# foundation-model-stack/fms-fsdp

Hardware: AMD Instinct MI355X
Metric: tokens/sec (aggregate) (higher is better)
Workload: dtype bf16; 1 GPU; model=llama2_7b, global_batch=2, seq_len=4096, parallelism=hsdp1

## Files before the change

fms_fsdp_amd/ops/hip/attention.hip:

```cpp
#include <cstdlib>
#include <cstring>

#include "common.h"
#include "attn_sched.h"
#include "attn_ws.h"

typedef __attribute__((ext_vector_type(8))) __bf16 bf16x8v;
typedef __attribute__((ext_vector_type(16))) float f32x16;
typedef __attribute__((ext_vector_type(4))) float f32x4v;

union U8 {
  bf16x8v v;
  unsigned u[4];
  bf16x8 s;
};

__device__ __forceinline__ unsigned pack2(float lo, float hi) {
  return ((unsigned)(unsigned short)f2bf(hi) << 16) |
         (unsigned short)f2bf(lo);
}

__device__ __forceinline__ bf16x8v pack_pT_chunk(const float* p) {
  unsigned w01 = pack2(p[0], p[1]);
  unsigned w23 = pack2(p[2], p[3]);
// ... 257 lines not shown
        pb1_1 = pack_pT_chunk(p + 8);
      }
    }
    __syncthreads();
    if (tile + 1 < ntiles) stage_k();
    if (act1) {
      const unsigned pvbase = pvb[cur] + 1024;
      U2x64 fr[2][2];
      tr_issue4<0, 128, 512, 640>(pvbase, fr[0][0], fr[0][1]);
#pragma unroll
      for (int t = 0; t < NT; ++t) {
        const int pp = t & 1;
        if (t + 1 < NT) {
          if (t + 1 == 1)
            tr_issue4<4096, 4096 + 128, 4096 + 512, 4096 + 640>(
                pvbase, fr[1][0], fr[1][1]);
          else if (t + 1 == 2)
            tr_issue4<8192, 8192 + 128, 8192 + 512, 8192 + 640>(
                pvbase, fr[0][0], fr[0][1]);
          else
            tr_issue4<12288, 12288 + 128, 12288 + 512, 12288 + 640>(
                pvbase, fr[1][0], fr[1][1]);
          tr_wait<4>(fr[pp][0], fr[pp][1]);
        } else {
          tr_wait<0>(fr[pp][0], fr[pp][1]);
        }
        accO[t] = __builtin_amdgcn_mfma_f32_32x32x16_bf16(fr[pp][0].v, pb1_0,
                                                          accO[t], 0, 0, 0);
        accO[t] = __builtin_amdgcn_mfma_f32_32x32x16_bf16(fr[pp][1].v, pb1_1,
                                                          accO[t], 0, 0, 0);
      }
    }
    __syncthreads();
    cur ^= 1;
  }

  const float inv_l = 1.f / l_run;
  short* op = og + ((long long)b * S * H + (long long)h) * D +
              (long long)my_q * qrow_stride;
#pragma unroll
  for (int t = 0; t < NT; ++t) {
#pragma unroll
    for (int g = 0; g < 4; ++g) {
      const int dv0 = t * 32 + 8 * g + 4 * hb;
      bf16x4 w;
#pragma unroll
      for (int j = 0; j < 4; ++j)
        w.v[j] = f2bf(accO[t][g * 4 + j] * inv_l);
      *(bf16x4*)(op + dv0) = w;
    }
  }
  if (hb == 0)
    lseg[((long long)bh) * S + my_q] =
        (m_run + __log2f(l_run)) * 0.6931471805599453f;
}
#undef KLDS
#undef VLDS

__global__ void attn_bwd_delta_kernel(const short* __restrict__ dog,
                                      const short* __restrict__ og,
                                      float* __restrict__ delta,
                                      int D, int S, int H, long long rows) {
  const long long row = ((long long)blockIdx.x * blockDim.x + threadIdx.x) / 64;
  if (row >= rows) return;
  const int lane = threadIdx.x & 63;
  const short* dop = dog + row * D;
  const short* op = og + row * D;
  float acc = 0.f;
  for (int i = lane * 2; i < D; i += 128) {
    acc += bf2f(dop[i]) * bf2f(op[i]) + bf2f(dop[i + 1]) * bf2f(op[i + 1]);
  }
  acc = wave_reduce_sum(acc);
  if (lane == 0) {
    const long long b = row / ((long long)S * H);
    const int si = (int)((row / H) % S);
    const int hi = (int)(row % H);
    delta[(b * H + hi) * (long long)S + si] = acc;
  }
}

template <int D>
__global__ __launch_bounds__(256, 2) void attn_bwd_dq_kernel(
    const short* __restrict__ kg, const short* __restrict__ dsw,
    short* __restrict__ dqg, int B, int S, int H, int KVH, int sched) {
  constexpr int KVB = 32;
  constexpr int NT = D / 32;
  extern __shared__ __attribute__((aligned(16))) char smem[];
  constexpr int KIMGB = KVB * D * 2;
  constexpr int SIMGB = KVB * 128 * 2;
#define KIMG(buf) (smem + ((buf) ? KIMGB + SIMGB : 0))
#define SIMG(buf) (smem + KIMGB + ((buf) ? KIMGB + SIMGB : 0))

  const int lane = threadIdx.x & 63;
  const int wid = threadIdx.x >> 6;
  const int col = lane & 31;
  const int hb = lane >> 5;

  const AttnWork wk = attn_sched_map(blockIdx.x, S / 128, B * H, sched, false);
  const int bh = __builtin_amdgcn_readfirstlane(wk.bh);
  const int b = bh / H;
  const int h = bh % H;
  const int kvh = h / (H / KVH);
  const int q0 = __builtin_amdgcn_readfirstlane(wk.tile) * 128;
  const int qw = q0 + wid * 32;
  const int my_q = qw + col;

  const long long qrow_stride = (long long)H * D;
  const long long krow_stride = (long long)KVH * D;
  const short* kbase = kg + ((long long)b * S * KVH + (long long)kvh) * D;
  const short* dsbase = dsw + (long long)bh * S * S + q0;

  f32x16 accDQ[NT];
#pragma unroll
  for (int t = 0; t < NT; ++t) accDQ[t] = (f32x16)(0.f);

  const int ntiles = (q0 + 128 + KVB - 1) / KVB;
  const int t256 = threadIdx.x;
  const int skey = t256 & 31;
  const int sgrp = t256 >> 5;
  const int skd0 = sgrp * (D / 8);
  const short* kp_s = kbase + (long long)skey * krow_stride + skd0;
  const long long kstep = (long long)KVB * krow_stride;
  const short* sp_s = dsbase + (long long)skey * S + sgrp * 16;
  const long long sstep = (long long)KVB * S;
  const int koff = SUBT_OFF(skey, skd0, 8);
  const int koff1 = SUBT_OFF(skey, skd0 + 8, 8);
  const int soff0 = SUBT_OFF(skey, sgrp * 16, 8);
  const int soff1 = SUBT_OFF(skey, sgrp * 16 + 8, 8);
  auto stage = [&](int buf) {
    if constexpr (D == 128) {
      *(f32x4*)(KIMG(buf) + koff) = *(const f32x4*)(kp_s);
      *(f32x4*)(KIMG(buf) + koff1) = *(const f32x4*)(kp_s + 8);
    } else {
      *(f32x4*)(KIMG(buf) + koff) = *(const f32x4*)(kp_s);
    }
    *(f32x4*)(SIMG(buf) + soff0) = *(const f32x4*)(sp_s);
    *(f32x4*)(SIMG(buf) + soff1) = *(const f32x4*)(sp_s + 8);
    kp_s += kstep;
    sp_s += sstep;
  };
  stage(0);
  __syncthreads();
  const unsigned ktr = tr_base<1024>(lane, col, hb);
  const unsigned kib[2] = {(unsigned)(unsigned long long)KIMG(0) + ktr,
                           (unsigned)(unsigned long long)KIMG(1) + ktr};
  const unsigned str = (unsigned)((((lane & 15) * 8) ^ (16 * hb)) +
                                  hb * 256 + ((col >> 4) << 10) +
                                  (wid * 32) * 64);
  const unsigned sib[2] = {(unsigned)(unsigned long long)SIMG(0) + str,
                           (unsigned)(unsigned long long)SIMG(1) + str};

  int cur = 0;
  for (int tile = 0; tile < ntiles; ++tile) {
    if (tile + 1 < ntiles) stage(cur ^ 1);
    U2x64 bs[2];
    tr_issue4<0, 128, 512, 512 + 128>(sib[cur], bs[0], bs[1]);
    tr_wait<0>(bs[0], bs[1]);
    const unsigned kbase_t = kib[cur];
    U2x64 fr[2][2];
    tr_issue4<0, 128, 512, 640>(kbase_t, fr[0][0], fr[0][1]);
#pragma unroll
    for (int t = 0; t < NT; ++t) {
      const int pp = t & 1;
      if (t + 1 < NT) {
        if (t + 1 == 1)
          tr_issue4<2048, 2048 + 128, 2048 + 512, 2048 + 640>(
              kbase_t, fr[1][0], fr[1][1]);
        else if (t + 1 == 2)
          tr_issue4<4096, 4096 + 128, 4096 + 512, 4096 + 640>(
              kbase_t, fr[0][0], fr[0][1]);
        else
          tr_issue4<6144, 6144 + 128, 6144 + 512, 6144 + 640>(
              kbase_t, fr[1][0], fr[1][1]);
        tr_wait<4>(fr[pp][0], fr[pp][1]);
      } else {
        tr_wait<0>(fr[pp][0], fr[pp][1]);
      }
      accDQ[t] = __builtin_amdgcn_mfma_f32_32x32x16_bf16(fr[pp][0].v,
                                                         bs[0].v, accDQ[t],
                                                         0, 0, 0);
      accDQ[t] = __builtin_amdgcn_mfma_f32_32x32x16_bf16(fr[pp][1].v,
                                                         bs[1].v, accDQ[t],
                                                         0, 0, 0);
    }
    __syncthreads();
    cur ^= 1;
  }

  short* dqp = dqg + ((long long)b * S * H + (long long)h) * D +
               (long long)my_q * qrow_stride;
#pragma unroll
  for (int t = 0; t < NT; ++t) {
#pragma unroll
    for (int g = 0; g < 4; ++g) {
      const int dk0 = t * 32 + 8 * g + 4 * hb;
      bf16x4 w;
#pragma unroll
      for (int j = 0; j < 4; ++j) w.v[j] = f2bf(accDQ[t][g * 4 + j]);
      *(bf16x4*)(dqp + dk0) = w;
    }
  }
}
#undef KIMG
#undef SIMG

template <int D>
// ... 283 lines not shown
      const int key = DROW(r, hb);
      *(short*)(my_p + key * 80 + col * 2) = f2bf(pv[r]);
    }
#define DKV_TRLOOP(ACC, A0, A1, BASE)                                        \
  do {                                                                       \
    _Pragma("unroll") for (int t = 0; t < NT; ++t) {                         \
      U2x64 f0, f1;                                                          \
      const unsigned b_t = (BASE) + t * 2048;                                \
      tr_issue4<0, 128, 512, 640>(b_t, f0, f1);                              \
      tr_wait<0>(f0, f1);                                                    \
      ACC[t] = __builtin_amdgcn_mfma_f32_32x32x16_bf16(A0, f0.v, ACC[t],     \
                                                       0, 0, 0);             \
      ACC[t] = __builtin_amdgcn_mfma_f32_32x32x16_bf16(A1, f1.v, ACC[t],     \
                                                       0, 0, 0);             \
    }                                                                        \
  } while (0)
    {
      bf16x8v pa[2];
#pragma unroll
      for (int kc = 0; kc < 2; ++kc) {
        const int inrow = kc * 32 + hb * 16;
        pa[kc] = *(const bf16x8v*)(my_p + col * 80 + inrow);
      }
      const unsigned dob = (unsigned)(unsigned long long)DOIMG(cur) + kv_swz;
      DKV_TRLOOP(accDV, pa[0], pa[1], dob);
    }
#pragma unroll
    for (int r = 0; r < 16; ++r) {
      const int key = DROW(r, hb);
      *(short*)(my_p + key * 80 + col * 2) = f2bf(ds[r]);
    }
    if constexpr (PUBLISH_DS) {
      const int key = lane & 31;
      const long long grow = ((long long)bh * S + kv0 + key) * S + q0;
#pragma unroll
      for (int c = 0; c < 2; ++c) {
        const int qc = ((lane >> 5) * 2 + c) * 8;
        *(f32x4*)(dsw + grow + qc) =
            *(const f32x4*)(my_p + key * 80 + qc * 2);
      }
    }
    {
      bf16x8v da[2];
#pragma unroll
      for (int kc = 0; kc < 2; ++kc) {
        const int inrow = kc * 32 + hb * 16;
        da[kc] = *(const bf16x8v*)(my_p + col * 80 + inrow);
      }
      const unsigned qib = (unsigned)(unsigned long long)QIMG(cur) + kv_swz;
      DKV_TRLOOP(accDK, da[0], da[1], qib);
    }
#undef DKV_TRLOOP
    __syncthreads();
    cur ^= 1;
  }
#undef QIMG
#undef DOIMG

#pragma unroll
  for (int t = 0; t < NT; ++t) {
#pragma unroll
    for (int r = 0; r < 16; ++r) {
      const int key_abs = kv0 + DROW(r, hb);
      const int feat = t * 32 + col;
      const long long off =
          ((long long)b * S + key_abs) * (long long)(KVH * D) +
          (long long)kvh * D + feat;
      const long long offv = ((long long)b * S + key_abs) * dvstride +
                             (long long)kvh * D + feat;
      if (OUT_BF16) {
        ((short*)dkg)[off] = f2bf(accDK[t][r]);
        ((short*)dvg)[offv] = f2bf(accDV[t][r]);
      } else if (ngrp > 1) {
        atomicAdd((float*)dkg + off, accDK[t][r]);
        atomicAdd((float*)dvg + offv, accDV[t][r]);
      } else {
        ((float*)dkg)[off] += accDK[t][r];
        ((float*)dvg)[offv] += accDV[t][r];
      }
    }
  }
}

static int g_attn_sched = -1;

static int attn_sched_get() {
  if (g_attn_sched < 0) {
    const char* e = getenv("FMS_AMD_ATTN_SCHED");
    g_attn_sched = (e && strcmp(e, "legacy") == 0) ? ATTN_SCHED_LEGACY
                                                   : ATTN_SCHED_BALANCED;
  }
  return g_attn_sched;
}

static long long g_attn_ws_limit = -1;

static long long attn_ws_limit_get() {
  if (g_attn_ws_limit < 0) {
    long long mb = ATTN_BWD_WS_DEFAULT_MB;
    const char* e = getenv("FMS_AMD_ATTN_BWD_WS_MB");
    if (e && *e) {
      char* end = nullptr;
      const long long val = strtoll(e, &end, 10);
      if (end != e && *end == '\0' && val >= 0 && val <= (1LL << 40)) mb = val;
    }
    g_attn_ws_limit = mb << 20;
  }
  return g_attn_ws_limit;
}

template <int D>
static void attn_bwd_launch(const void* do_, const void* q, const void* k,
                            const void* v, const float* lse, void* dq,
                            void* dk, void* dv, float* delta_ws, void* ds_ws,
                            int B, int S, int H, int KVH, float scale,
                            int out_bf16, long long vstride,
                            long long dvstride, hipStream_t stream) {
  const unsigned grid = (unsigned)(S / 128) * (unsigned)(B * H);
  const int sched = attn_sched_get();
  const int lds_dkv = 4 * 32 * D * 2 + 4 * 32 * D * 2 + 4 * 32 * 80;
#define DKV_LAUNCH(OUT, PUB)                                                  \
  attn_bwd_dkv_kernel<D, OUT, PUB><<<grid, 256, lds_dkv, stream>>>(           \
      (const short*)do_, (const short*)q, (const short*)k, (const short*)v,   \
      lse, delta_ws, dk, dv, (short*)ds_ws, B, S, H, KVH, scale, vstride,     \
      dvstride, sched)
  if (ds_ws) {
    if (out_bf16)
      DKV_LAUNCH(true, true);
    else
      DKV_LAUNCH(false, true);
    const int lds_dq = 2 * (32 * D * 2 + 32 * 128 * 2);
    attn_bwd_dq_kernel<D><<<grid, 256, lds_dq, stream>>>(
        (const short*)k, (const short*)ds_ws, (short*)dq, B, S, H, KVH, sched);
  } else {
    if (out_bf16)
      DKV_LAUNCH(true, false);
    else
      DKV_LAUNCH(false, false);
    const int lds_dq = 2 * (32 * D * 2 + 32 * D * 2);
    attn_bwd_dq_recompute_kernel<D><<<grid, 256, lds_dq, stream>>>(
        (const short*)do_, (const short*)q, (const short*)k, (const short*)v,
        lse, delta_ws, (short*)dq, B, S, H, KVH, scale, vstride, sched);
  }
#undef DKV_LAUNCH
}

extern "C" {

long long attn_bwd_ws_limit(long long bytes) {
  const long long prev = attn_ws_limit_get();
  if (bytes >= 0) g_attn_ws_limit = bytes;
  return prev;
}

int attn_sched_mode(int mode) {
  const int prev = attn_sched_get();
  if (mode >= 0) g_attn_sched = mode;
  return prev;
}

void launch_attn_fwd(const void* q, const void* k, const void* v, void* o,
                     float* lse, int B, int S, int H, int KVH, int D,
                     float scale, long long vstride, hipStream_t stream) {
  const unsigned grid = (unsigned)(S / 128) * (unsigned)(B * H);
  const int sched = attn_sched_get();
  const int lds = 3 * 64 * D * 2;
  if (D == 128)
    attn_fwd_kernel<128><<<grid, 256, lds, stream>>>(
        (const short*)q, (const short*)k, (const short*)v, (short*)o, lse, B,
        S, H, KVH, scale, vstride, sched);
  else
    attn_fwd_kernel<64><<<grid, 256, lds, stream>>>(
        (const short*)q, (const short*)k, (const short*)v, (short*)o, lse, B,
        S, H, KVH, scale, vstride, sched);
}

void launch_attn_bwd(const void* do_, const void* q, const void* k,
                     const void* v, const void* o, const float* lse, void* dq,
                     void* dk, void* dv, float* delta_ws, void* ds_ws,
                     int B, int S, int H,
                     int KVH, int D, float scale, int out_bf16,
                     long long vstride, long long dvstride,
                     hipStream_t stream) {
  const long long rows = (long long)B * S * H;
  attn_bwd_delta_kernel<<<(int)((rows * 64 + 255) / 256), 256, 0, stream>>>(
      (const short*)do_, (const short*)o, delta_ws, D, S, H, rows);
  if (D == 128)
    attn_bwd_launch<128>(do_, q, k, v, lse, dq, dk, dv, delta_ws, ds_ws, B, S,
                         H, KVH, scale, out_bf16, vstride, dvstride, stream);
  else
    attn_bwd_launch<64>(do_, q, k, v, lse, dq, dk, dv, delta_ws, ds_ws, B, S,
                        H, KVH, scale, out_bf16, vstride, dvstride, stream);
}

}
```

fms_fsdp_amd/ops/hip/bindings.cpp:

```cpp
#include <torch/extension.h>
#include <c10/hip/HIPStream.h>
#include <hip/hip_runtime_api.h>

#include <string>
#include <tuple>
#include <vector>

#include "attn_ws.h"

using torch::Tensor;

extern "C" {
void launch_rmsnorm_fwd(const void*, const void*, void*, float*, int, int,
                        float, hipStream_t);
void launch_rmsnorm_bwd(const void*, const void*, const void*, const float*,
                        const void*, void*, float*, int, int, hipStream_t);
void launch_add_rmsnorm_fwd(const void*, const void*, const void*, void*,
                            void*, float*, int, int, float, hipStream_t);
void launch_rope(const void*, void*, const float*, const float*, int, int,
                 int, int, int, long long, long long, hipStream_t);
void launch_swiglu_fwd(const void*, void*, long long, int, hipStream_t);
void launch_swiglu_bwd(const void*, const void*, void*, long long, int,
                       hipStream_t);
void launch_ce_fwd_bwd(void*, const long long*, float*, const float*,
                       long long, int, int, hipStream_t);
void launch_adamw(float*, const void*, int, float*, float*, void*, int,
                  long long, float, float, float, float, float, float, float,
                  const float*, hipStream_t);
void launch_sqnorm(const void*, int, float*, long long, hipStream_t);
void launch_attn_fwd(const void*, const void*, const void*, void*, float*,
                     int, int, int, int, int, float, long long, hipStream_t);
void launch_attn_bwd(const void*, const void*, const void*, const void*,
                     const void*, const float*, void*, void*, void*, float*,
                     void*, int, int, int, int, int, float, int,
                     long long, long long, hipStream_t);
int attn_sched_mode(int);
long long attn_bwd_ws_limit(long long);
void launch_cconv_fwd(const void*, const void*, const float*, void*, int,
                      int, int, int, hipStream_t);
void launch_cconv_bwd(const void*, const void*, const void*, const float*,
                      void*, void*, float*, float*, int, int, int, int,
                      hipStream_t);
int launch_gemm_nt(const void*, const void*, void*, int, int, int,
                   hipStream_t);
void launch_segsum_exp_fwd(const float*, void*, long long, int, hipStream_t);
void launch_segsum_exp_bwd(const void*, const float*, float*, long long, int,
                           hipStream_t);
void launch_ssd_prep_fwd(const void*, const float*, const float*, float*,
                         float*, long long, int, int, long long, hipStream_t);
void launch_ssd_prep_bwd(const float*, const float*, const void*,
                         const float*, const float*, void*, float*, float*,
                         long long, int, int, long long, long long,
                         hipStream_t);
void launch_ssd_xdt_fwd(const void*, const float*, const float*, void*, void*,
                        long long, int, int, int, long long, hipStream_t);
void launch_ssd_xdt_bwd(const void*, const void*, const void*, const float*,
                        const float*, void*, float*, float*, long long, int,
                        int, int, long long, long long, hipStream_t);
void launch_ssd_sl_fwd(const float*, const void*, void*, long long, int, int,
                       int, hipStream_t);
void launch_ssd_sl_bwd(const void*, const void*, const float*, void*, float*,
                       long long, int, int, int, hipStream_t);
void launch_ssd_ygate_fwd(const void*, const void*, const float*, const void*,
                          const float*, const void*, void*, long long, int,
                          int, int, int, long long, long long, hipStream_t);
void launch_ssd_ygate_bwd(const void*, const void*, const void*, const float*,
                          const void*, const float*, const void*, void*,
                          void*, float*, void*, float*, void*, long long, int,
                          int, int, int, long long, long long, long long,
                          long long, hipStream_t);
}

static hipStream_t cur_stream() {
  return c10::hip::getCurrentHIPStream().stream();
}

#define CHECK_BF16_CONTIG(t)                                        \
  TORCH_CHECK(t.scalar_type() == torch::kBFloat16, #t " must be bf16"); \
  TORCH_CHECK(t.is_contiguous(), #t " must be contiguous");

std::tuple<Tensor, Tensor> rmsnorm_fwd(Tensor x, Tensor w, double eps) {
  CHECK_BF16_CONTIG(x);
  CHECK_BF16_CONTIG(w);
  const int rows = x.size(0), H = x.size(1);
  TORCH_CHECK(H % 8 == 0, "H must be divisible by 8");
  auto y = torch::empty_like(x);
  auto rinv = torch::empty({rows}, x.options().dtype(torch::kFloat32));
  launch_rmsnorm_fwd(x.data_ptr(), w.data_ptr(), y.data_ptr(),
                     rinv.data_ptr<float>(), rows, H, (float)eps,
                     cur_stream());
  return {y, rinv};
}

std::tuple<Tensor, Tensor> rmsnorm_bwd(Tensor dy, Tensor x, Tensor w,
                                       Tensor rinv,
                                       c10::optional<Tensor> dextra) {
  CHECK_BF16_CONTIG(dy);
  CHECK_BF16_CONTIG(x);
  const int rows = x.size(0), H = x.size(1);
  auto dx = torch::empty_like(x);
  auto dw = torch::zeros({H}, x.options().dtype(torch::kFloat32));
  launch_rmsnorm_bwd(dy.data_ptr(), x.data_ptr(), w.data_ptr(),
                     rinv.data_ptr<float>(),
                     dextra.has_value() ? dextra->data_ptr() : nullptr,
                     dx.data_ptr(), dw.data_ptr<float>(), rows, H,
                     cur_stream());
  return {dx, dw};
}

std::tuple<Tensor, Tensor, Tensor> add_rmsnorm_fwd(Tensor x, Tensor res,
                                                   Tensor w, double eps) {
  CHECK_BF16_CONTIG(x);
  CHECK_BF16_CONTIG(res);
  const int rows = x.size(0), H = x.size(1);
  auto y = torch::empty_like(x);
  auto s_out = torch::empty_like(x);
  auto rinv = torch::empty({rows}, x.options().dtype(torch::kFloat32));
  launch_add_rmsnorm_fwd(x.data_ptr(), res.data_ptr(), w.data_ptr(),
                         y.data_ptr(), s_out.data_ptr(),
// ... 43 lines not shown
Tensor swiglu_fwd(Tensor gu) {
  CHECK_BF16_CONTIG(gu);
  const long long rows = gu.size(0);
  const int H2 = gu.size(1);
  TORCH_CHECK(H2 % 16 == 0);
  auto h = torch::empty({rows, H2 / 2}, gu.options());
  launch_swiglu_fwd(gu.data_ptr(), h.data_ptr(), rows, H2 / 2, cur_stream());
  return h;
}

Tensor swiglu_bwd(Tensor dy, Tensor gu) {
  CHECK_BF16_CONTIG(dy);
  CHECK_BF16_CONTIG(gu);
  const long long rows = gu.size(0);
  const int H2 = gu.size(1);
  auto dgu = torch::empty_like(gu);
  launch_swiglu_bwd(dy.data_ptr(), gu.data_ptr(), dgu.data_ptr(), rows,
                    H2 / 2, cur_stream());
  return dgu;
}

void ce_fwd_bwd(Tensor logits, Tensor labels, Tensor loss_sum, Tensor denom,
                int64_t ignore_index) {
  CHECK_BF16_CONTIG(logits);
  TORCH_CHECK(labels.scalar_type() == torch::kInt64 && labels.is_contiguous());
  const int rows = logits.size(0), V = logits.size(1);
  launch_ce_fwd_bwd(logits.data_ptr(),
                    reinterpret_cast<const long long*>(labels.data_ptr<int64_t>()),
                    loss_sum.data_ptr<float>(), denom.data_ptr<float>(),
                    (long long)ignore_index, rows, V, cur_stream());
}

void adamw(Tensor p, Tensor g, Tensor m, Tensor v, double step, double lr,
           double b1, double b2, double eps, double wd,
           c10::optional<Tensor> grad_scale,
           c10::optional<Tensor> p_bf16_out) {
  TORCH_CHECK(p.scalar_type() == torch::kFloat32 && p.is_contiguous());
  const long long n = p.numel();
  TORCH_CHECK(n % 4 == 0, "shard size must be divisible by 4");
  auto dt_code = [](torch::ScalarType t) {
    if (t == torch::kBFloat16) return 1;
    if (t == torch::kFloat16) return 2;
    TORCH_CHECK(t == torch::kFloat32, "dtype must be fp32/bf16/fp16");
    return 0;
  };
  const int gdt = dt_code(g.scalar_type());
  int odt = 0;
  if (p_bf16_out.has_value()) {
    odt = dt_code(p_bf16_out->scalar_type());
    TORCH_CHECK(odt != 0, "low-precision publish target must be bf16/fp16");
  }
  const float bc1 = 1.f - powf((float)b1, (float)step);
  const float bc2 = 1.f - powf((float)b2, (float)step);
  launch_adamw(p.data_ptr<float>(), g.data_ptr(), gdt, m.data_ptr<float>(),
               v.data_ptr<float>(),
               p_bf16_out.has_value() ? p_bf16_out->data_ptr() : nullptr, odt,
               n,
               (float)lr, (float)b1, (float)b2, (float)eps, (float)wd, bc1,
               bc2,
               grad_scale.has_value() ? grad_scale->data_ptr<float>() : nullptr,
               cur_stream());
}

void sq_norm_accum(Tensor t, Tensor out) {
  TORCH_CHECK(t.is_contiguous());
  const long long n = t.numel();
  TORCH_CHECK(n % 4 == 0);
  const int dt = t.scalar_type() == torch::kBFloat16 ? 1
                 : t.scalar_type() == torch::kFloat16 ? 2 : 0;
  launch_sqnorm(t.data_ptr(), dt, out.data_ptr<float>(), n, cur_stream());
}

std::string attn_sched_mode_py(c10::optional<std::string> mode) {
  int m = -1;
  if (mode.has_value()) {
    TORCH_CHECK(*mode == "balanced" || *mode == "legacy",
                "attn_sched_mode: expected 'balanced' or 'legacy', got '",
                *mode, "'");
    m = (*mode == "legacy") ? 1 : 0;
  }
  return attn_sched_mode(m) == 1 ? "legacy" : "balanced";
}

int64_t attn_bwd_ws_limit_py(c10::optional<int64_t> bytes) {
  long long v = -1;
  if (bytes.has_value()) {
    TORCH_CHECK(*bytes >= 0, "attn_bwd_ws_limit: expected bytes >= 0, got ",
                *bytes);
    v = *bytes;
  }
  return attn_bwd_ws_limit(v);
}

std::tuple<Tensor, Tensor> attn_fwd(Tensor q, Tensor k, Tensor v) {
  CHECK_BF16_CONTIG(q);
  CHECK_BF16_CONTIG(k);
  const long long vs = row_stride4(v);
  const int b = q.size(0), s = q.size(1), h = q.size(2), d = q.size(3);
  const int kvh = k.size(2);
  TORCH_CHECK(d == 64 || d == 128, "head_dim must be 64 or 128");
  TORCH_CHECK(s % 128 == 0, "seq len must be a multiple of 128");
  auto o = torch::empty_like(q);
  auto lse = torch::empty({b, h, s}, q.options().dtype(torch::kFloat32));
  const float scale = 1.f / sqrtf((float)d);
  launch_attn_fwd(q.data_ptr(), k.data_ptr(), v.data_ptr(), o.data_ptr(),
                  lse.data_ptr<float>(), b, s, h, kvh, d, scale, vs,
                  cur_stream());
  return {o, lse};
}

std::tuple<Tensor, Tensor, Tensor> attn_bwd(Tensor do_, Tensor q, Tensor k,
                                            Tensor v, Tensor o, Tensor lse,
                                            c10::optional<Tensor> dv_out) {
  CHECK_BF16_CONTIG(do_);
  const long long vs = row_stride4(v);
  const int b = q.size(0), s = q.size(1), h = q.size(2), d = q.size(3);
  const int kvh = k.size(2);
  auto dq = torch::empty_like(q);
  const bool out_bf16 = (kvh == h);
  auto opts = q.options().dtype(out_bf16 ? torch::kBFloat16 : torch::kFloat32);
  auto dk = out_bf16 ? torch::empty({b, s, kvh, d}, opts)
                     : torch::zeros({b, s, kvh, d}, opts);
  Tensor dv;
  long long dvs = (long long)kvh * d;
  if (dv_out.has_value() && out_bf16) {
    dv = *dv_out;
    dvs = row_stride4(dv);
  } else {
    dv = out_bf16 ? torch::empty({b, s, kvh, d}, opts)
                  : torch::zeros({b, s, kvh, d}, opts);
  }
  auto delta = torch::empty({b, h, s}, q.options().dtype(torch::kFloat32));
  Tensor ds_ws;
  if (attn_bwd_use_workspace(b, h, s, attn_bwd_ws_limit(-1)))
    ds_ws = torch::empty({(long long)b * h, (long long)s, (long long)s},
                         q.options());
  const float scale = 1.f / sqrtf((float)d);
  launch_attn_bwd(do_.data_ptr(), q.data_ptr(), k.data_ptr(), v.data_ptr(),
                  o.data_ptr(), lse.data_ptr<float>(), dq.data_ptr(),
                  dk.data_ptr(), dv.data_ptr(), delta.data_ptr<float>(),
                  ds_ws.defined() ? ds_ws.data_ptr() : nullptr, b, s,
                  h, kvh, d, scale, out_bf16 ? 1 : 0, vs, dvs, cur_stream());
  if (out_bf16) return {dq, dk, dv};
  return {dq, dk.to(torch::kBFloat16), dv.to(torch::kBFloat16)};
}

Tensor cconv_fwd(Tensor x, Tensor w, Tensor bias) {
  CHECK_BF16_CONTIG(x);
  CHECK_BF16_CONTIG(w);
  const int b = x.size(0), l = x.size(1), c = x.size(2);
  const int W = w.size(1);
  TORCH_CHECK(c % 8 == 0 && W >= 2 && W <= 4);
  TORCH_CHECK(bias.scalar_type() == torch::kFloat32);
  auto y = torch::empty_like(x);
  launch_cconv_fwd(x.data_ptr(), w.data_ptr(), bias.data_ptr<float>(),
                   y.data_ptr(), b * l, l, c, W, cur_stream());
  return y;
}

std::tuple<Tensor, Tensor, Tensor> cconv_bwd(Tensor dy, Tensor x, Tensor w,
                                             Tensor bias) {
  CHECK_BF16_CONTIG(dy);
  CHECK_BF16_CONTIG(x);
  const int b = x.size(0), l = x.size(1), c = x.size(2);
  const int W = w.size(1);
  TORCH_CHECK(c % 8 == 0 && W >= 2 && W <= 4);
// ... 130 lines not shown
  return out;
}

std::tuple<Tensor, Tensor> ssd_sl_bwd(Tensor g, Tensor scores, Tensor dacs,
                                      int64_t H, int64_t G) {
  const long long N = dacs.size(0);
  const int Q = dacs.size(1);
  auto dsh = torch::empty({N, (long long)Q, (long long)Q}, g.options());
  auto dcs = torch::zeros_like(dacs);
  launch_ssd_sl_bwd(g.data_ptr(), scores.data_ptr(), dacs.data_ptr<float>(),
                    dsh.data_ptr(), dcs.data_ptr<float>(), N, (int)H, (int)G,
                    Q, cur_stream());
  return {dsh, dcs};
}

Tensor ssd_ygate_fwd(Tensor ydiag, Tensor yoff, Tensor dacs, Tensor x,
                     Tensor Dp, Tensor z, int64_t H, int64_t G, int64_t P,
                     int64_t Q) {
  const long long sx = slice_stride(x, "x");
  const long long sz = slice_stride(z, "z");
  TORCH_CHECK(ydiag.is_contiguous() && yoff.is_contiguous());
  const long long rows = x.size(0);
  auto out = torch::empty({rows, H * P}, x.options().dtype(torch::kBFloat16));
  launch_ssd_ygate_fwd(ydiag.data_ptr(), yoff.data_ptr(),
                       dacs.data_ptr<float>(), x.data_ptr(),
                       Dp.data_ptr<float>(), z.data_ptr(), out.data_ptr(),
                       rows * H * P / 8, (int)H, (int)G, (int)Q, (int)P, sx,
                       sz, cur_stream());
  return out;
}

std::vector<Tensor> ssd_ygate_bwd(Tensor dout, Tensor ydiag, Tensor yoff,
                                  Tensor dacs, Tensor x, Tensor Dp, Tensor z,
                                  int64_t H, int64_t G, int64_t P,
                                  int64_t Q) {
  const long long sx = slice_stride(x, "x");
  const long long sz = slice_stride(z, "z");
  const long long rows = x.size(0);
  auto o = x.options().dtype(torch::kBFloat16);
  auto dydiag = torch::empty({rows, H * P}, o);
  auto dyoff = torch::empty({rows, H * P}, o);
  auto ddacs = torch::empty_like(dacs);
  auto dx = torch::empty({rows, H * P}, o);
  auto dD_rows = torch::empty({rows, H}, x.options().dtype(torch::kFloat32));
  auto dz = torch::empty({rows, H * P}, o);
  launch_ssd_ygate_bwd(dout.data_ptr(), ydiag.data_ptr(), yoff.data_ptr(),
                       dacs.data_ptr<float>(), x.data_ptr(),
                       Dp.data_ptr<float>(), z.data_ptr(), dydiag.data_ptr(),
                       dyoff.data_ptr(), ddacs.data_ptr<float>(),
                       dx.data_ptr(), dD_rows.data_ptr<float>(),
                       dz.data_ptr(), rows * H, (int)H, (int)G, (int)Q,
                       (int)P, sx, sz, H * P, H * P, cur_stream());
  return {dydiag, dyoff, ddacs, dx, dD_rows, dz};
}

PYBIND11_MODULE(TORCH_EXTENSION_NAME, mod) {
  mod.def("segsum_exp_fwd", &segsum_exp_fwd);
  mod.def("segsum_exp_bwd", &segsum_exp_bwd);
  mod.def("cconv_fwd", &cconv_fwd);
  mod.def("cconv_bwd", &cconv_bwd);
  mod.def("rmsnorm_fwd", &rmsnorm_fwd);
  mod.def("rmsnorm_bwd", &rmsnorm_bwd);
  mod.def("add_rmsnorm_fwd", &add_rmsnorm_fwd);
  mod.def("rope_fwd", &rope_fwd);
  mod.def("rope_into", &rope_into);
  mod.def("swiglu_fwd", &swiglu_fwd);
  mod.def("swiglu_bwd", &swiglu_bwd);
  mod.def("ce_fwd_bwd", &ce_fwd_bwd);
  mod.def("adamw", &adamw);
  mod.def("sq_norm_accum", &sq_norm_accum);
  mod.def("gemm_nt", &gemm_nt);
  mod.def("ssd_prep_fwd", &ssd_prep_fwd);
  mod.def("ssd_prep_bwd", &ssd_prep_bwd);
  mod.def("ssd_xdt_fwd", &ssd_xdt_fwd);
  mod.def("ssd_xdt_bwd", &ssd_xdt_bwd);
  mod.def("ssd_sl_fwd", &ssd_sl_fwd);
  mod.def("ssd_sl_bwd", &ssd_sl_bwd);
  mod.def("ssd_ygate_fwd", &ssd_ygate_fwd);
  mod.def("ssd_ygate_bwd", &ssd_ygate_bwd);
  mod.def("attn_fwd", &attn_fwd);
  mod.def("attn_bwd", &attn_bwd);
  mod.def("attn_sched_mode", &attn_sched_mode_py,
          pybind11::arg("mode") = pybind11::none());
  mod.def("attn_bwd_ws_limit", &attn_bwd_ws_limit_py,
          pybind11::arg("bytes") = pybind11::none());
}
```

Baseline: 22170 tokens/s.

## Add key-lane dK/dV backward kernel with tiled dS workspace layout

Adds a new attention backward dK/dV kernel in which each lane owns one key. V is held in registers, and dO/Q tiles are read with LDS transpose loads (ds_read_b64_tr_b16) for the dV and dK MFMAs. The kernel writes dS into a tiled 32x32 block layout, and the dQ kernel gains an addressing mode that reads this layout contiguously. It is selected by default through a new env/python mode switch. The aim is less LDS traffic and better-coalesced dS publishing in the backward pass, at the cost of extra kernel complexity and a layout coupling between the two kernels.

```diff
diff --git a/fms_fsdp_amd/ops/hip/attention.hip b/fms_fsdp_amd/ops/hip/attention.hip
--- a/fms_fsdp_amd/ops/hip/attention.hip
+++ b/fms_fsdp_amd/ops/hip/attention.hip
@@ -363,7 +363,8 @@
 template <int D>
 __global__ __launch_bounds__(256, 2) void attn_bwd_dq_kernel(
     const short* __restrict__ kg, const short* __restrict__ dsw,
-    short* __restrict__ dqg, int B, int S, int H, int KVH, int sched) {
+    short* __restrict__ dqg, int B, int S, int H, int KVH, int sched,
+    int ws_tiled) {
   constexpr int KVB = 32;
   constexpr int NT = D / 32;
   extern __shared__ __attribute__((aligned(16))) char smem[];
@@ -402,7 +403,11 @@
   const int skd0 = sgrp * (D / 8);
   const short* kp_s = kbase + (long long)skey * krow_stride + skd0;
   const long long kstep = (long long)KVB * krow_stride;
-  const short* sp_s = dsbase + (long long)skey * S + sgrp * 16;
+  const short* sp_s =
+      ws_tiled ? dsw + (long long)bh * S * S +
+                     (long long)(q0 / 32 + (sgrp >> 1)) * 1024 +
+                     (sgrp & 1) * 512 + skey * 16
+               : dsbase + (long long)skey * S + sgrp * 16;
   const long long sstep = (long long)KVB * S;
   const int koff = SUBT_OFF(skey, skd0, 8);
   const int koff1 = SUBT_OFF(skey, skd0 + 8, 8);
@@ -852,6 +857,283 @@
   }
 }
 
+template <int O>
+__device__ __forceinline__ void tr_issue4x2(unsigned b0, unsigned b1,
+                                            U2x64& r0, U2x64& r1) {
+  asm volatile(
+      "ds_read_b64_tr_b16 %0, %4 offset:%c6\n\t"
+      "ds_read_b64_tr_b16 %1, %5 offset:%c7\n\t"
+      "ds_read_b64_tr_b16 %2, %4 offset:%c8\n\t"
+      "ds_read_b64_tr_b16 %3, %5 offset:%c9"
+      : "=&v"(r0.u[0]), "=&v"(r0.u[1]), "=&v"(r1.u[0]), "=&v"(r1.u[1])
+      : "v"(b0), "v"(b1), "i"(O), "i"(O + 256), "i"(O + 512), "i"(O + 768)
+      : "memory");
+}
+
+__device__ __forceinline__ void kl_issue(int t, unsigned b0, unsigned b1,
+                                         U2x64& r0, U2x64& r1) {
+  switch (t) {
+    case 0: tr_issue4x2<0>(b0, b1, r0, r1); break;
+    case 1: tr_issue4x2<2048>(b0, b1, r0, r1); break;
+    case 2: tr_issue4x2<4096>(b0, b1, r0, r1); break;
+    default: tr_issue4x2<6144>(b0, b1, r0, r1); break;
+  }
+}
+
+__device__ __forceinline__ bf16x8v pack_slice(const float* p) {
+  U8 b;
+  b.u[0] = pack2(p[0], p[1]);
+  b.u[1] = pack2(p[2], p[3]);
+  b.u[2] = pack2(p[4], p[5]);
+  b.u[3] = pack2(p[6], p[7]);
+  return b.v;
+}
+
+template <int D, bool OUT_BF16, bool PUBLISH_DS>
+__global__ __launch_bounds__(256, D == 64 ? 3 : 2) void
+attn_bwd_dkv_keylane_kernel(
+    const short* __restrict__ dog, const short* __restrict__ qg,
+    const short* __restrict__ kg, const short* __restrict__ vg,
+    const float* __restrict__ lseg, const float* __restrict__ deltag,
+    void* __restrict__ dkg, void* __restrict__ dvg,
+    short* __restrict__ dsw, int B, int S, int H,
+    int KVH, float scale, long long vstride, long long dvstride, int sched,
+    int ws_tiled) {
+  constexpr int KVB = 32;
+  constexpr int NC = D / 16;
+  constexpr int NT = D / 32;
+  extern __shared__ __attribute__((aligned(16))) char smem[];
+  char* k_lds = smem;
+  constexpr int IMGB = 32 * D * 2;
+#define QIMG(buf) (smem + 4 * KVB * D * 2 + ((buf) ? 2 * IMGB : 0))
+#define DOIMG(buf) (smem + 4 * KVB * D * 2 + IMGB + ((buf) ? 2 * IMGB : 0))
+  float* rowc = (float*)(smem + 4 * KVB * D * 2 + 4 * IMGB);
+
+  const int lane = threadIdx.x & 63;
+  const int wid = __builtin_amdgcn_readfirstlane(threadIdx.x >> 6);
+  const int col = lane & 31;
+  const int hb = lane >> 5;
+
+  const AttnWork wk = attn_sched_map(blockIdx.x, S / 128, B * H, sched, true);
+  const int bh = __builtin_amdgcn_readfirstlane(wk.bh);
+  const int tile = __builtin_amdgcn_readfirstlane(wk.tile);
+  const int b = bh / H;
+  const int h = bh % H;
+  const int kvh = h / (H / KVH);
+  const int ngrp = H / KVH;
+  const int kv0 = tile * 128 + wid * KVB;
+
+  const long long qrow_stride = (long long)H * D;
+  const long long krow_stride = (long long)KVH * D;
+  const short* qbase = qg + ((long long)b * S * H + (long long)h) * D;
+  const short* dobase = dog + ((long long)b * S * H + (long long)h) * D;
+  const short* kbase = kg + ((long long)b * S * KVH + (long long)kvh) * D;
+  const short* vbase = vg + (long long)b * S * vstride + (long long)kvh * D;
+
+  char* my_k = k_lds + wid * KVB * D * 2;
+
+  {
+    constexpr int CHUNKS = KVB * D / 8;
+    for (int i = lane; i < CHUNKS; i += 64) {
+      const int row = i / (D / 8);
+      const int cb = (i % (D / 8)) * 8;
+      const long long g = (long long)(kv0 + row) * krow_stride + cb;
+      *(f32x4*)(my_k + SUBT_OFF(row, cb, 8)) = *(const f32x4*)(kbase + g);
+    }
+  }
+  bf16x8v vreg[NC];
+  {
+    const short* vp = vbase + (long long)(kv0 + col) * vstride + hb * 8;
+#pragma unroll
+    for (int c = 0; c < NC; ++c) vreg[c] = *(const bf16x8v*)(vp + c * 16);
+  }
+
+  f32x16 accDV[NT], accDK[NT];
+#pragma unroll
+  for (int t = 0; t < NT; ++t) {
+    accDV[t] = (f32x16)(0.f);
+    accDK[t] = (f32x16)(0.f);
+  }
+
+  const int q_start = tile * 128;
+  const int t256 = threadIdx.x;
+  const int sq = t256 & 31;
+  const int sd0 = (t256 >> 5) * ((D == 128) ? 16 : 8);
+  const short* qp_s = qbase + (long long)q_start * qrow_stride;
+  const short* dop_s = dobase + (long long)q_start * qrow_stride;
+  const int goff = sq * (int)qrow_stride + sd0;
+  const long long qstep = 32 * qrow_stride;
+  const int soff0 = SUBT_OFF(sq, sd0, 8);
+  const int soff1 = SUBT_OFF(sq, sd0 + 8, 8);
+  const int rcw = wid & 1;
+  const float* rc_s = (rcw ? deltag : lseg) + (long long)bh * S + q_start;
+  const float rc_mul = rcw ? 1.0f : 1.4426950408889634f;
+  f32x4v qpre0, qpre1, dpre0, dpre1;
+  float rcpre = 0.f;
+#define DKV_FETCH()                                   \
+  do {                                                \
+    qpre0 = *(const f32x4v*)(qp_s + goff);            \
+    dpre0 = *(const f32x4v*)(dop_s + goff);           \
+    if constexpr (D == 128) {                         \
+      qpre1 = *(const f32x4v*)(qp_s + goff + 8);      \
+      dpre1 = *(const f32x4v*)(dop_s + goff + 8);     \
+    }                                                 \
+    rcpre = rc_s[col];                                \
+  } while (0)
+#define DKV_ADVANCE(on)                               \
+  do {                                                \
+    qp_s += (on) ? qstep : 0;                         \
+    dop_s += (on) ? qstep : 0;                        \
+    rc_s += (on) ? 32 : 0;                            \
+  } while (0)
+#define DKV_COMMIT(buf)                               \
+  do {                                                \
+    *(f32x4v*)(QIMG(buf) + soff0) = qpre0;            \
+    *(f32x4v*)(DOIMG(buf) + soff0) = dpre0;           \
+    if constexpr (D == 128) {                         \
+      *(f32x4v*)(QIMG(buf) + soff1) = qpre1;          \
+      *(f32x4v*)(DOIMG(buf) + soff1) = dpre1;         \
+    }                                                 \
+    rowc[(buf) * 64 + rcw * 32 + col] = rcpre * rc_mul; \
+  } while (0)
+  DKV_FETCH();
+  DKV_COMMIT(0);
+  __syncthreads();
+
+  const unsigned tr0 =
+      (unsigned)((lane & 15) * 8 + hb * 128 + (col >> 4) * 1024);
+  const unsigned tr1 = tr0 ^ 16u;
+  const float scale2 = scale * 1.4426950408889634f;
+  const int key = kv0 + col;
+  const int pub_off = ws_tiled ? col * 16 + hb * 8 : col * S + hb * 8;
+  const int pub_kc = ws_tiled ? 512 : 16;
+  const int pub_qmul = ws_tiled ? 32 : 1;
+  short* pub_base =
+      dsw + (long long)bh * S * S +
+      (ws_tiled ? (long long)(kv0 / 32) * S * 32 : (long long)kv0 * S);
+
+  int cur = 0;
+  for (int q0 = q_start; q0 < S; q0 += 32) {
+    const bool more = q0 + 32 < S;
+
+    f32x16 accS = (f32x16)(0.f), accDP = (f32x16)(0.f);
+#pragma unroll
+    for (int c = 0; c < NC; ++c) {
+      const int boff = SUBT_OFF(col, c * 16 + hb * 8, 8);
+      const bf16x8v ka = *(const bf16x8v*)(my_k + boff);
+      const bf16x8v qbf = *(const bf16x8v*)(QIMG(cur) + boff);
+      const bf16x8v dbf = *(const bf16x8v*)(DOIMG(cur) + boff);
+      accS = __builtin_amdgcn_mfma_f32_32x32x16_bf16(qbf, ka, accS, 0, 0, 0);
+      accDP = __builtin_amdgcn_mfma_f32_32x32x16_bf16(dbf, vreg[c], accDP,
+                                                      0, 0, 0);
+    }
+
+    const f32x4v* lse4 = (const f32x4v*)(rowc + cur * 64) + hb;
+    const f32x4v* del4 = (const f32x4v*)(rowc + cur * 64 + 32) + hb;
+    const unsigned dob = (unsigned)(unsigned long long)DOIMG(cur);
+    const unsigned qib = (unsigned)(unsigned long long)QIMG(cur);
+    float pv[16], ds[16];
+#pragma unroll
+    for (int g = 0; g < 4; ++g) {
+      const f32x4v lse_q2 = lse4[2 * g];
+      const f32x4v delta_q = del4[2 * g];
+#pragma unroll
+      for (int j = 0; j < 4; ++j) {
+        const int r = g * 4 + j;
+        const int q = q0 + DROW(r, hb);
+        float pval = exp2f(accS[r] * scale2 - lse_q2[j]);
+        if (key > q) pval = 0.f;
+        pv[r] = pval;
+        ds[r] = pval * (accDP[r] - delta_q[j]) * scale;
+      }
+    }
+    const bf16x8v pb0 = pack_slice(pv), pb1 = pack_slice(pv + 8);
+    const bf16x8v db0 = pack_slice(ds), db1 = pack_slice(ds + 8);
+
+    __builtin_amdgcn_sched_barrier(0);
+    DKV_ADVANCE(more);
+    DKV_FETCH();
+    __builtin_amdgcn_sched_barrier(0);
+
+    if constexpr (PUBLISH_DS) {
+      short* grow = pub_base + (long long)q0 * pub_qmul;
+      *(bf16x8v*)(grow + pub_off) = pack_pT_chunk(ds);
+      *(bf16x8v*)(grow + pub_off + pub_kc) = pack_pT_chunk(ds + 8);
+    }
+
+    __builtin_amdgcn_sched_barrier(0);
+
+    U2x64 fr[2][2];
+    kl_issue(0, dob + tr0, dob + tr1, fr[0][0], fr[0][1]);
+#define DKV_KLLOOP(ACC, B0, B1, BASE, NEXT_ISSUE)                            \
+  do {                                                                       \
+    _Pragma("unroll") for (int t = 0; t < NT; ++t) {                         \
+      const int pp = t & 1;                                                  \
+      if (t + 1 < NT) {                                                      \
+        kl_issue(t + 1, (BASE) + tr0, (BASE) + tr1, fr[pp ^ 1][0],           \
+                 fr[pp ^ 1][1]);                                             \
+        tr_wait<4>(fr[pp][0], fr[pp][1]);                                    \
+      } else {                                                               \
+        NEXT_ISSUE;                                                          \
+      }                                                                      \
+      ACC[t] = __builtin_amdgcn_mfma_f32_32x32x16_bf16(fr[pp][0].v, B0,      \
+                                                       ACC[t], 0, 0, 0);     \
+      ACC[t] = __builtin_amdgcn_mfma_f32_32x32x16_bf16(fr[pp][1].v, B1,      \
+                                                       ACC[t], 0, 0, 0);     \
+    }                                                                        \
+  } while (0)
+    DKV_KLLOOP(accDV, pb0, pb1, dob,
+               (kl_issue(0, qib + tr0, qib + tr1, fr[0][0], fr[0][1]),
+                tr_wait<4>(fr[1][0], fr[1][1])));
+    DKV_KLLOOP(accDK, db0, db1, qib, (tr_wait<0>(fr[1][0], fr[1][1])));
+#undef DKV_KLLOOP
+
+    DKV_COMMIT(cur ^ 1);
+    __syncthreads();
+    cur ^= 1;
+  }
+#undef DKV_FETCH
+#undef DKV_ADVANCE
+#undef DKV_COMMIT
+#undef QIMG
+#undef DOIMG
+
+  auto flush = [&](const f32x16& acc, int t, void* outg, long long rstride) {
+    __builtin_amdgcn_wave_barrier();
+#pragma unroll
+    for (int g = 0; g < 4; ++g) {
+      f32x4v w;
+#pragma unroll
+      for (int j = 0; j < 4; ++j) w[j] = acc[g * 4 + j];
+      *(f32x4v*)(my_k + col * 128 + (((2 * g + hb) ^ (col & 7)) * 16)) = w;
+    }
+    __builtin_amdgcn_wave_barrier();
+    const long long ubase = ((long long)b * S + kv0) * rstride +
+                            (long long)kvh * D + t * 32;
+    const int loff = 4 * hb * (int)rstride + col;
+#pragma unroll
+    for (int r = 0; r < 16; ++r) {
+      const int krel = DROW(r, hb);
+      const float val = *(const float*)(my_k + krel * 128 +
+                                        (((col >> 2) ^ (krel & 7)) * 16) +
+                                        (col & 3) * 4);
+      const long long uoff = ubase + (long long)DROW(r, 0) * rstride;
+      if (OUT_BF16) {
+        ((short*)outg + uoff)[loff] = f2bf(val);
+      } else if (ngrp > 1) {
+        atomicAdd((float*)outg + uoff + loff, val);
+      } else {
+        ((float*)outg + uoff)[loff] += val;
+      }
+    }
+  };
+#pragma unroll
+  for (int t = 0; t < NT; ++t) {
+    flush(accDK[t], t, dkg, (long long)(KVH * D));
+    flush(accDV[t], t, dvg, dvstride);
+  }
+}
+
 static int g_attn_sched = -1;
 
 static int attn_sched_get() {
@@ -877,6 +1159,19 @@
     g_attn_ws_limit = mb << 20;
   }
   return g_attn_ws_limit;
+}
+
+#define ATTN_DKV_KEYLANE 0
+#define ATTN_DKV_LEGACY 1
+static int g_attn_dkv = -1;
+
+static int attn_dkv_get() {
+  if (g_attn_dkv < 0) {
+    const char* e = getenv("FMS_AMD_ATTN_DKV");
+    g_attn_dkv = (e && strcmp(e, "legacy") == 0) ? ATTN_DKV_LEGACY
+                                                 : ATTN_DKV_KEYLANE;
+  }
+  return g_attn_dkv;
 }
 
 template <int D>
@@ -888,12 +1183,23 @@
                             long long dvstride, hipStream_t stream) {
   const unsigned grid = (unsigned)(S / 128) * (unsigned)(B * H);
   const int sched = attn_sched_get();
-  const int lds_dkv = 4 * 32 * D * 2 + 4 * 32 * D * 2 + 4 * 32 * 80;
+  const bool keylane = attn_dkv_get() == ATTN_DKV_KEYLANE;
+  const int ws_tiled = keylane;
+  const int lds_dkv =
+      4 * 32 * D * 2 + 4 * 32 * D * 2 + (keylane ? 2 * 64 * 4 : 4 * 32 * 80);
+#define DKV_ARGS                                                              \
+  (const short*)do_, (const short*)q, (const short*)k, (const short*)v, lse,  \
+      delta_ws, dk, dv, (short*)ds_ws, B, S, H, KVH, scale, vstride,          \
+      dvstride, sched
 #define DKV_LAUNCH(OUT, PUB)                                                  \
-  attn_bwd_dkv_kernel<D, OUT, PUB><<<grid, 256, lds_dkv, stream>>>(           \
-      (const short*)do_, (const short*)q, (const short*)k, (const short*)v,   \
-      lse, delta_ws, dk, dv, (short*)ds_ws, B, S, H, KVH, scale, vstride,     \
-      dvstride, sched)
+  do {                                                                        \
+    if (keylane)                                                              \
+      attn_bwd_dkv_keylane_kernel<D, OUT, PUB>                                \
+          <<<grid, 256, lds_dkv, stream>>>(DKV_ARGS, ws_tiled);               \
+    else                                                                      \
+      attn_bwd_dkv_kernel<D, OUT, PUB>                                        \
+          <<<grid, 256, lds_dkv, stream>>>(DKV_ARGS);                         \
+  } while (0)
   if (ds_ws) {
     if (out_bf16)
       DKV_LAUNCH(true, true);
@@ -901,7 +1207,8 @@
       DKV_LAUNCH(false, true);
     const int lds_dq = 2 * (32 * D * 2 + 32 * 128 * 2);
     attn_bwd_dq_kernel<D><<<grid, 256, lds_dq, stream>>>(
-        (const short*)k, (const short*)ds_ws, (short*)dq, B, S, H, KVH, sched);
+        (const short*)k, (const short*)ds_ws, (short*)dq, B, S, H, KVH, sched,
+        ws_tiled);
   } else {
     if (out_bf16)
       DKV_LAUNCH(true, false);
@@ -913,6 +1220,7 @@
         lse, delta_ws, (short*)dq, B, S, H, KVH, scale, vstride, sched);
   }
 #undef DKV_LAUNCH
+#undef DKV_ARGS
 }
 
 extern "C" {
@@ -926,6 +1234,12 @@
 int attn_sched_mode(int mode) {
   const int prev = attn_sched_get();
   if (mode >= 0) g_attn_sched = mode;
+  return prev;
+}
+
+int attn_dkv_mode(int mode) {
+  const int prev = attn_dkv_get();
+  if (mode >= 0) g_attn_dkv = mode;
   return prev;
 }
 
diff --git a/fms_fsdp_amd/ops/hip/bindings.cpp b/fms_fsdp_amd/ops/hip/bindings.cpp
--- a/fms_fsdp_amd/ops/hip/bindings.cpp
+++ b/fms_fsdp_amd/ops/hip/bindings.cpp
@@ -35,6 +35,7 @@
                      void*, int, int, int, int, int, float, int,
                      long long, long long, hipStream_t);
 int attn_sched_mode(int);
+int attn_dkv_mode(int);
 long long attn_bwd_ws_limit(long long);
 void launch_cconv_fwd(const void*, const void*, const float*, void*, int,
                       int, int, int, hipStream_t);
@@ -244,6 +245,17 @@
   return attn_sched_mode(m) == 1 ? "legacy" : "balanced";
 }
 
+std::string attn_dkv_mode_py(c10::optional<std::string> mode) {
+  int m = -1;
+  if (mode.has_value()) {
+    TORCH_CHECK(*mode == "keylane" || *mode == "legacy",
+                "attn_dkv_mode: expected 'keylane' or 'legacy', got '", *mode,
+                "'");
+    m = (*mode == "legacy") ? 1 : 0;
+  }
+  return attn_dkv_mode(m) == 1 ? "legacy" : "keylane";
+}
+
 int64_t attn_bwd_ws_limit_py(c10::optional<int64_t> bytes) {
   long long v = -1;
   if (bytes.has_value()) {
@@ -540,6 +552,8 @@
   mod.def("attn_bwd", &attn_bwd);
   mod.def("attn_sched_mode", &attn_sched_mode_py,
           pybind11::arg("mode") = pybind11::none());
+  mod.def("attn_dkv_mode", &attn_dkv_mode_py,
+          pybind11::arg("mode") = pybind11::none());
   mod.def("attn_bwd_ws_limit", &attn_bwd_ws_limit_py,
           pybind11::arg("bytes") = pybind11::none());
 }
```

Measured after the change: 22780 tokens/s (median of 6 runs). 2.8% higher.
